# ZhangHH233/Retinal_OCT_Image_Segmentation_via_Deep_Learning

Measured on AMD Instinct MI355X. Metric: B-scans/sec (train fwd+bwd) at batch 32, 512x1024, higher is better.
Workload: dtype bf16; 1 GPU; SOTAS/Layers_Segment UNet(1,8,init_features=32) train step, 512x1024, batch 32/GPU (BASELINE configs[1]); global_batch=32, parallelism=dp1, hip_graph=False

## Files before the change

include/oct_hip.h:

```cpp
#ifndef OCT_HIP_H
#define OCT_HIP_H

#include <stddef.h>
#include <stdint.h>

#ifdef __cplusplus
extern "C" {
#endif

#define OCT_VERSION 220

#define OCT_DT_BF16 0
#define OCT_DT_F32 1

#define OCT_OK 0
#define OCT_IMG_SHIFT_ALL 2
#define OCT_E_INVALID (-22)
#define OCT_E_LAUNCH (-5)
#define OCT_E_NODEVICE (-19)

#define OCT_XF_NONE 0
#define OCT_XF_AFFINE_RELU 1
#define OCT_XF_AFFINE 2

// ... 69 lines not shown
  int kh, kw;
  int depth;
  int in_img_shift;
  int dy_img_mul, dy_img_add;
  int partials;
} OctWgradDesc;
typedef struct OctWgradArgs {
  const void* x0; const void* x1;
  const float* scale0; const float* shift0;
  const float* scale1; const float* shift1;
  const void* dy;
  float* dwp;
  float* dbias;
  const void* dy_y; const float* dy_coef; const float* dy_scale; const float* dy_shift;
  float* dbias_partials;
  void* dy_out;
} OctWgradArgs;
int oct_conv_wgrad(const OctWgradDesc* d, const OctWgradArgs* a, void* stream);
int oct_conv_wgrad_partials(const OctWgradDesc* d);
int oct_reduce_bias_partials(const float* part, int nparts, int rows, int channels, float* dbias, int accumulate,
                             void* stream);
int oct_conv_wgrad_fused_apply_ok(const OctWgradDesc* d);
int oct_conv_wgrad_apply_store_ok(const OctWgradDesc* d);
int oct_conv_wgrad_all_depth_taps_ok(const OctWgradDesc* d);
typedef struct OctConvBwdFusedArgs {
  const void* x;
  const float* scale; const float* shift;
  const float* mean; const float* invstd;
  const void* dy;
  const void* wpacked;
  void* dx;
  float* dwp;
  float* partials;
} OctConvBwdFusedArgs;
int oct_conv_backward_fused_ok(const OctWgradDesc* d);
int oct_conv_backward_fused_blocks(const OctWgradDesc* d);
int oct_conv_backward_fused(const OctWgradDesc* d, const OctConvBwdFusedArgs* a, void* stream);
int oct_unpack_wgrad(int mode, const float* dwp, float* grad, int cout, int cin, int accumulate, void* stream);
int oct_unpack_wgrad_kk(const float* dwp, float* grad, int cout, int cin, int kh, int kw, int accumulate, void* stream);
int oct_unpack_wgrad3d(int mode, const float* dwp, float* grad, int cout, int cin, int kdi, int accumulate, void* stream);
typedef struct OctUnpackJob {
  int mode, cout, cin, accumulate;
  int nparts, reserved;
  const float* dwp;
  float* grad;
} OctUnpackJob;
// ... 337 lines not shown
```

retinal_oct_image_segmentation_via_deep_learning_amd/_lib.py:

```python
from __future__ import annotations

import ctypes as C
import os
import subprocess
import threading

PKG_DIR = os.path.dirname(os.path.abspath(__file__))
LIB_PATH = os.environ.get("OCT_HIP_LIB") or os.path.join(PKG_DIR, "liboct_hip.so")
CSRC_DIR = os.path.join(PKG_DIR, "csrc")

DT_BF16, DT_F32 = 0, 1
XF_NONE, XF_AFFINE_RELU, XF_AFFINE = 0, 1, 2
IN_PLAIN, IN_S2D = 0, 1
IMG_SHIFT_ALL = 2
ACT_NONE, ACT_RELU, ACT_SIGMOID = 0, 1, 2
ACT_PRELU = 3
OUT_PLAIN, OUT_D2S = 0, 1
PACK_CONV_FPROP, PACK_CONV_DGRAD, PACK_DECONV_FPROP, PACK_DECONV_DGRAD, PACK_1X1_DGRAD, PACK_1X1_FPROP = range(6)
PACK_CONV3D_FPROP, PACK_CONV3D_DGRAD, PACK_DECONV3D_FPROP, PACK_DECONV3D_DGRAD = 6, 7, 8, 9
MAX_CLASSES = 16
HEAD_LOSS_SLOTS = 2 + 3 * MAX_CLASSES
SEG_NHWC, SEG_NCHW = 0, 1

c_void_p, c_int, c_size_t, c_float, c_double = C.c_void_p, C.c_int, C.c_size_t, C.c_float, C.c_double
# ... 120 lines not shown
    "oct_depth_pool_fwd": (c_int, [c_int, c_void_p, c_void_p, c_size_t, c_size_t, c_void_p]),
    "oct_depth_pool_bwd": (c_int, [c_int, c_void_p, c_void_p, c_void_p, c_size_t, c_size_t, c_void_p]),
    "oct_pack_weights_kk": (c_int, [c_int, c_int, c_void_p, c_void_p, c_int, c_int, c_int, c_int, c_void_p]),
    "oct_unpack_wgrad_kk": (c_int, [c_void_p, c_void_p, c_int, c_int, c_int, c_int, c_int, c_void_p]),
    "oct_affine_prelu_fwd": (c_int, [c_int, c_void_p, c_void_p, c_void_p, c_void_p, c_void_p, c_size_t, c_int, c_void_p]),
    "oct_affine_prelu_bwd": (c_int, [c_int, c_void_p, c_void_p, c_void_p, c_void_p, c_void_p, c_void_p, c_void_p, c_size_t,
                                     c_int, c_void_p]),
    "oct_maxpool_idx_fwd": (c_int, [c_int, c_void_p, c_void_p, c_void_p, c_int, c_int, c_int, c_int, c_int, c_void_p]),
    "oct_index_scatter": (c_int, [c_int, c_void_p, c_void_p, c_void_p, c_int, c_size_t, c_size_t, c_int, c_void_p]),
    "oct_index_gather": (c_int, [c_int, c_void_p, c_void_p, c_void_p, c_int, c_size_t, c_size_t, c_int, c_void_p]),
    "oct_prelu_bn_fused_ok": (c_int, [c_int, c_int]),
    "oct_dact_bn_reduce_prelu": (c_int, [c_int, c_void_p, c_void_p, c_void_p, c_void_p, c_void_p, c_void_p, c_void_p, c_void_p, c_void_p,
                                         c_int, c_int, c_int, c_int, c_void_p]),
    "oct_bn_bwd_apply_prelu_to": (c_int, [c_int, c_void_p, c_void_p, c_void_p, c_void_p, c_void_p, c_void_p, c_void_p, c_size_t, c_int,
                                          c_void_p]),
    "oct_maxpool_code_fwd": (c_int, [c_int, c_void_p, c_void_p, c_void_p, c_int, c_int, c_int, c_int, c_int, c_void_p]),
    "oct_window_scatter": (c_int, [c_int, c_void_p, c_void_p, c_void_p, c_int, c_int, c_int, c_int, c_int, c_void_p]),
    "oct_window_gather": (c_int, [c_int, c_void_p, c_void_p, c_void_p, c_int, c_int, c_int, c_int, c_int, c_void_p]),
    "oct_pack_weights_batch": (c_int, [c_int, c_int, C.POINTER(PackJob), c_void_p]),
    "oct_conv_forward": (c_int, [C.POINTER(ConvDesc), C.POINTER(ConvArgs), c_void_p]),
    "oct_conv_wgrad": (c_int, [C.POINTER(WgradDesc), C.POINTER(WgradArgs), c_void_p]),
    "oct_conv_wgrad_fused_apply_ok": (c_int, [C.POINTER(WgradDesc)]),
    "oct_conv_wgrad_apply_store_ok": (c_int, [C.POINTER(WgradDesc)]),
    "oct_conv_wgrad_all_depth_taps_ok": (c_int, [C.POINTER(WgradDesc)]),
    "oct_conv_backward_fused_ok": (c_int, [C.POINTER(WgradDesc)]),
    "oct_conv_backward_fused_blocks": (c_int, [C.POINTER(WgradDesc)]),
    "oct_conv_backward_fused": (c_int, [C.POINTER(WgradDesc), C.POINTER(ConvBwdFusedArgs), c_void_p]),
    "oct_conv_wgrad_partials": (c_int, [C.POINTER(WgradDesc)]),
    "oct_reduce_bias_partials": (c_int, [c_void_p, c_int, c_int, c_int, c_void_p, c_int, c_void_p]),
    "oct_unpack_wgrad": (c_int, [c_int, c_void_p, c_void_p, c_int, c_int, c_int, c_void_p]),
    "oct_unpack_wgrad_batch": (c_int, [c_int, C.POINTER(UnpackJob), c_void_p]),
    "oct_bn_finalize": (c_int, [c_void_p, c_int, c_int, c_double, c_void_p, c_void_p, c_float, c_float,
                                c_void_p, c_void_p, c_void_p, c_void_p, c_void_p, c_void_p, c_void_p, c_void_p]),
    "oct_bn_eval_coeffs": (c_int, [c_int, c_void_p, c_void_p, c_void_p, c_void_p, c_float, c_void_p, c_void_p,
                                   c_void_p, c_void_p]),
    "oct_bn_relu_pool_fwd": (c_int, [c_int, c_void_p, c_void_p, c_void_p, c_void_p, c_int, c_int, c_int, c_int,
                                     c_void_p]),
    "oct_bn_relu_fwd": (c_int, [c_int, c_void_p, c_void_p, c_void_p, c_void_p, c_size_t, c_int, c_void_p]),
    "oct_dact_bn_reduce": (c_int, [c_int, c_void_p, c_void_p, c_void_p, c_void_p, c_void_p, c_void_p, c_void_p,
                                   c_void_p, c_void_p, c_int, c_int, c_int, c_int, c_void_p]),
    "oct_dact_bn_reduce_blocks": (c_int, [c_int, c_int, c_int, c_int, c_int]),
    "oct_bn_bwd_apply_pool_ok": (c_int, [c_int, c_int, c_int, c_int, c_int]),
    "oct_bn_bwd_apply_pool": (c_int, [c_int, c_void_p, c_void_p, c_void_p, c_void_p, c_void_p, c_void_p, c_void_p,
                                      c_int, c_int, c_int, c_int, c_void_p]),
    "oct_bn_bwd_finalize": (c_int, [c_void_p, c_int, c_int, c_double, c_void_p, c_void_p, c_void_p, c_void_p,
                                    c_void_p, c_void_p, c_int, c_void_p]),
# ... 151 lines not shown
```

retinal_oct_image_segmentation_via_deep_learning_amd/csrc/common.h:

```cpp
#pragma once
#include <hip/hip_runtime.h>
#include <stdint.h>
#include <stddef.h>
#include "../../include/oct_hip.h"

typedef __bf16 bf16_t;
typedef float f32x16 __attribute__((ext_vector_type(16)));
typedef float f32x4 __attribute__((ext_vector_type(4)));
typedef __bf16 bf16x8 __attribute__((ext_vector_type(8)));
typedef __bf16 bf16x4 __attribute__((ext_vector_type(4)));
typedef unsigned int u32x4 __attribute__((ext_vector_type(4)));
typedef unsigned int u32x2 __attribute__((ext_vector_type(2)));

void oct_set_error(const char* fmt, ...);
#define OCT_CHECK(cond, ...)            \
  do {                                  \
    if (!(cond)) {                      \
      oct_set_error(__VA_ARGS__);       \
      return OCT_E_INVALID;             \
    }                                   \
  } while (0)
int oct_check_launch(const char* what);
int oct_lds_optin(const void* kernel, int bytes);
constexpr int OCT_LDS_CAP = 160 * 1024;
// ... 13 lines not shown
bool gemm1_plan(const OctConvDesc* d, ConvPlan* pl);
void igemm_plan(const OctConvDesc* d, ConvPlan* pl);
int launch_first(const ConvPlan& pl, const OctConvDesc* d, const OctConvArgs* a, hipStream_t s);
int launch_roll3d(const ConvPlan& pl, const OctConvDesc* d, const OctConvArgs* a, hipStream_t s);
int launch_igemm2(const ConvPlan& pl, const OctConvDesc* d, const OctConvArgs* a, hipStream_t s);
int launch_gemm1(const ConvPlan& pl, const OctConvDesc* d, const OctConvArgs* a, hipStream_t s);
int launch_igemm(const ConvPlan& pl, const OctConvDesc* d, const OctConvArgs* a, hipStream_t s);
bool igemm2_fused_plan(const OctWgradDesc* d, ConvPlan* pl);
int launch_igemm2_fused(const ConvPlan& pl, const OctWgradDesc* d, const OctConvBwdFusedArgs* a, hipStream_t s);

enum WgradPath { WGRAD_FIRST, WGRAD_W2, WGRAD_GENERIC };
struct WgradPlan {
  WgradPath path;
  int kernel;
  int cb, ib, th;
  int grid;
  int slabs;
  bool all_depth_taps;
};
bool first_wgrad_plan(const OctWgradDesc* d, bool dbias, bool dy_coef, WgradPlan* pl);
bool wgrad2_plan(const OctWgradDesc* d, WgradPlan* pl);
void wgrad_plan(const OctWgradDesc* d, WgradPlan* pl);
bool wgrad2_apply_store_ok(const OctWgradDesc* d, const WgradPlan& pl);
int launch_first_wgrad(const WgradPlan& pl, const OctWgradDesc* d, const OctWgradArgs* a, hipStream_t s);
int launch_wgrad2(const WgradPlan& pl, const OctWgradDesc* d, const OctWgradArgs* a, hipStream_t s);
int launch_wgrad(const WgradPlan& pl, const OctWgradDesc* d, const OctWgradArgs* a, hipStream_t s);

__device__ __forceinline__ float xf_floor(int xf) { return xf == 2 ? -__builtin_inff() : 0.f; }
__device__ __forceinline__ float to_f32(float v) { return v; }
__device__ __forceinline__ float to_f32(bf16_t v) { return (float)v; }
template <typename T> __device__ __forceinline__ T from_f32(float v);
template <> __device__ __forceinline__ float from_f32<float>(float v) { return v; }
template <> __device__ __forceinline__ bf16_t from_f32<bf16_t>(float v) { return (bf16_t)v; }
__device__ __forceinline__ unsigned pack_bf16x2(float a, float b) {
  typedef __bf16 bf16x2 __attribute__((ext_vector_type(2)));
  bf16x2 v;
  v[0] = (bf16_t)a;
  v[1] = (bf16_t)b;
  return __builtin_bit_cast(unsigned, v);
}
__device__ __forceinline__ float bf16lo(unsigned u) { return __uint_as_float(u << 16); }
__device__ __forceinline__ float bf16hi(unsigned u) { return __uint_as_float(u & 0xffff0000u); }

template <typename T, int V> struct alignas((sizeof(T) * V) > 16 ? 16 : (sizeof(T) * V)) VecT { T v[V]; };

template <typename T, int V>
// ... 179 lines not shown
```

retinal_oct_image_segmentation_via_deep_learning_amd/csrc/conv_dispatch.hip:

```cpp
#include "common.h"
#include <stdlib.h>

static bool v2_enabled() {
  static const bool on = [] { const char* e = getenv("OCT_DISABLE_V2"); return !(e && e[0] == '1'); }();
  return on;
}

static ConvPlan plan_conv_forward(const OctConvDesc* d) {
  ConvPlan pl = {};
  if (v2_enabled()) {
    if (first_plan(d, &pl) || roll3d_plan(d, &pl)) return pl;
    if (igemm2_plan(d, &pl)) {
      gemm1_plan(d, &pl);
      return pl;
    }
  }
  igemm_plan(d, &pl);
  return pl;
}

static WgradPlan plan_conv_wgrad(const OctWgradDesc* d, bool dbias, bool dy_coef) {
  WgradPlan pl = {};
  if (v2_enabled() && (first_wgrad_plan(d, dbias, dy_coef, &pl) || wgrad2_plan(d, &pl))) return pl;
  wgrad_plan(d, &pl);
// ... 93 lines not shown
  OCT_CHECK(!(d->xform1 && (!a->scale1 || !a->shift1)), "oct_conv_wgrad: xform1 without scale/shift");
  OCT_CHECK(!d->partials || !a->dbias || a->dbias_partials, "oct_conv_wgrad: partials mode with a bias gradient needs dbias_partials");
  const bool apply_store = a->dy_coef && a->dy_out;
  OCT_CHECK(!a->dy_out || a->dy_coef, "oct_conv_wgrad: dy_out goes with dy_coef");
  OCT_CHECK(!apply_store || oct_conv_wgrad_apply_store_ok(d),
            "oct_conv_wgrad: dy_coef + dy_out is not available for this descriptor (oct_conv_wgrad_apply_store_ok)");
  OCT_CHECK(!apply_store || !a->dbias, "oct_conv_wgrad: dy_coef + dy_out takes no bias gradient");
  const WgradPlan pl = plan_conv_wgrad(d, a->dbias != nullptr, a->dy_coef != nullptr && !apply_store);
  OCT_CHECK(!a->dy_coef || apply_store || pl.path == WGRAD_FIRST, "oct_conv_wgrad: the fused BN-backward apply is only implemented for the 1->F first layer in bf16");
  OCT_CHECK(!a->dy_coef || (a->dy_y && a->dy_scale && a->dy_shift), "oct_conv_wgrad: fused apply needs y, scale, shift");
  if (d->partials) {
    const int slabs = plan_conv_wgrad(d, false, false).slabs;
    OCT_CHECK(pl.slabs == slabs, "oct_conv_wgrad: with these arguments the launch writes %d partial slabs, oct_conv_wgrad_partials "
              "answered %d (first layer with a bias gradient?)", pl.slabs, slabs);
  }
  hipStream_t s = as_stream(stream);
  switch (pl.path) {
    case WGRAD_FIRST: return launch_first_wgrad(pl, d, a, s);
    case WGRAD_W2: return launch_wgrad2(pl, d, a, s);
    default: return launch_wgrad(pl, d, a, s);
  }
}

static bool plan_conv_backward_fused(const OctWgradDesc* d, ConvPlan* pl) {
  return d && v2_enabled() && igemm2_fused_plan(d, pl);
}

extern "C" int oct_conv_backward_fused_ok(const OctWgradDesc* d) {
  ConvPlan pl;
  return plan_conv_backward_fused(d, &pl) ? 1 : 0;
}

extern "C" int oct_conv_backward_fused_blocks(const OctWgradDesc* d) {
  ConvPlan pl;
  return plan_conv_backward_fused(d, &pl) ? pl.stat_rows : 0;
}

extern "C" int oct_conv_backward_fused(const OctWgradDesc* d, const OctConvBwdFusedArgs* a, void* stream) {
  OCT_CHECK(d && a, "oct_conv_backward_fused: null descriptor");
  ConvPlan pl;
  OCT_CHECK(plan_conv_backward_fused(d, &pl),
            "oct_conv_backward_fused: not available for this descriptor (oct_conv_backward_fused_ok): bf16, 2-D, 3x3, c0 = cout = 32, "
            "c1 = 0, BN + ReLU on load, w %% 32 == 0, h %% 8 == 0, atomics mode");
  OCT_CHECK(a->x && a->scale && a->shift && a->mean && a->invstd && a->dy && a->wpacked && a->dx && a->dwp && a->partials,
            "oct_conv_backward_fused: null tensor");
  return launch_igemm2_fused(pl, d, a, as_stream(stream));
// ... 2 lines not shown
```

retinal_oct_image_segmentation_via_deep_learning_amd/csrc/wgrad2.hip:

```cpp
#include "common.h"

#include <type_traits>

struct Wgrad2Params {
  const bf16_t* x0; const bf16_t* x1;
  const float* sc0; const float* sh0; const float* sc1; const float* sh1;
  const bf16_t* dy; float* dwp; float* dbias;
  int n, h, w, c0, c1, ktot, cout, xf0, xf1, dy_mode;
  int tiles_x, tiles_y, ntiles, per_wg;
  int interleave;
  int depth, img_shift;
  int dy_mul, dy_add;
  int part_mode; size_t slab_elems; float* dbias_part;
  int ty0, pad_y, nstore;
  unsigned long long* trace;
  const bf16_t* dy_y; const float* dy_coef; const float* dy_sc; const float* dy_sh; bf16_t* dy_out;
};

#ifdef OCT_TRACE
#define W2TRACE(slot, idx)                                                                                     \
  do {                                                                                                         \
    if (p.trace && blockIdx.x == 0 && blockIdx.y == 0 && blockIdx.z == 0 && (threadIdx.x & 63) == 0 && (idx) < 256) \
      p.trace[(slot) * 256 + (idx)] = __builtin_amdgcn_s_memtime();                                            \
  } while (0)
// ... 64 lines not shown
    const bool second = cg >= p.c0;
    const bool xf = second ? (p.xf1 != 0) : (p.xf0 != 0);
    sxf[i] = xf ? (second ? p.sc1[cg - p.c0] : p.sc0[cg]) : 1.f;
    sxf[32 * IB + i] = xf ? (second ? p.sh1[cg - p.c0] : p.sh0[cg]) : 0.f;
  }
  float* const sdy = reinterpret_cast<float*>(smem + w2_sdy(TAPS, CB, IB, TH));
  if constexpr (DYAPPLY) {
    for (int i = tid; i < 32 * CB; i += 512) {
      const int ch = co_sb + i;
      sdy[i] = p.dy_coef[ch]; sdy[32 * CB + i] = p.dy_coef[p.cout + ch]; sdy[2 * 32 * CB + i] = p.dy_coef[2 * p.cout + ch];
      sdy[3 * 32 * CB + i] = p.dy_sc[ch]; sdy[4 * 32 * CB + i] = p.dy_sh[ch];
    }
  }
  __syncthreads();

  if (wave >= 4) {
    const int ptid = tid - 256, g = ptid & 3, pb = ptid >> 2;
    constexpr int SIB = (NPI * 4 + 255) / 256;
    constexpr int SDB = (NPD * 4 + 255) / 256;
    constexpr int D = DRING;
    typedef typename std::conditional<DYAPPLY, W2StageY<CB, SDB>, W2NoY>::type StageY;
    struct Stage { u32x4 ri[IB][SIB]; u32x4 rd[CB][SDB]; unsigned vm[IB]; unsigned vd; int img, tyi, txi; StageY yy; };
    Stage R[D];
    int reli[SIB], reld[SDB];
    int lyv[RSH ? SIB : 1];
    unsigned code[SIB], dcode[SDB];
#pragma unroll
    for (int j = 0; j < SIB; ++j) {
      const int pix = pb + 64 * j;
      const int ly = pix / LW, lx = pix - ly * LW;
      reli[j] = (RSH ? ly + p.ty0 : ly) * p.w + lx;
      if constexpr (RSH) lyv[j] = ly;
      const int ylast = p.h - (p.tiles_y - 1) * TH + HALO_Y, xlast = p.w - (p.tiles_x - 1) * TW + HALO;
      unsigned c = pix >= NPI ? 16u : 0u;
      if (HALO) c |= ((!RSH && HALO_Y && ly == 0) ? 1u : 0u) | (lx == 0 ? 4u : 0u);
      c |= ((!RSH && ly >= ylast) ? 2u : 0u) | (lx >= xlast ? 8u : 0u);
      code[j] = c | (SWZ ? (unsigned)(((lx >> 3) & 1) << 1) << 8 : 0u);
    }
    unsigned dswz[SDB];
#pragma unroll
    for (int j = 0; j < SDB; ++j) {
      const int pix = pb + 64 * j;
      const int ly = pix / TW, lx = pix - ly * TW;
      dswz[j] = SWZ ? (unsigned)(((lx >> 3) & 1) << 1) : 0u;
      reld[j] = (p.dy_mode == OCT_IN_S2D) ? (2 * ly) * (2 * p.w) + 2 * lx : ly * p.w + lx;
      dcode[j] = RAGGED ? ((ly >= p.h - (p.tiles_y - 1) * TH ? 2u : 0u) | (lx >= p.w - (p.tiles_x - 1) * TW ? 8u : 0u)) : 0u;
    }
    auto issue = [&](int s, Stage& S) {
      int t = t0 + s * tstep;
      const int txi = t % p.tiles_x; t /= p.tiles_x;
      const int tyi = t % p.tiles_y; const int img = t / p.tiles_y;
      const unsigned edge = 16u | (tyi == 0 ? 1u : 0u) | (tyi == p.tiles_y - 1 ? 2u : 0u) | (txi == 0 ? 4u : 0u) |
                            (txi == p.tiles_x - 1 ? 8u : 0u);
      const size_t origin = ((size_t)img * p.h + tyi * TH) * p.w + txi * TW;
      S.img = img; S.tyi = tyi; S.txi = txi;
      int ylo = 0; unsigned ynum = 0;
      if constexpr (RSH) {
        const int ytop = tyi * TH - p.pad_y + p.ty0;
        ylo = max(0, -ytop);
        ynum = (unsigned)max(0, min(LH, p.h - ytop) - ylo);
      }
      bool zok = true;
      size_t in_origin = origin;
      if (D3 && p.depth > 0) {
        const int dz = img % p.depth + p.img_shift;
        zok = dz >= 0 && dz < p.depth;
        if (zok) in_origin = ((size_t)(img + p.img_shift) * p.h + tyi * TH) * p.w + txi * TW;
      }
#pragma unroll
      for (int blk = 0; blk < IB; ++blk) {
        const int cg = ci_sb + blk * 32;
        const bool second = cg >= p.c0;
        const int cs = second ? p.c1 : p.c0;
        const bf16_t* base = second ? p.x1 + in_origin * p.c1 + (cg - p.c0) : p.x0 + in_origin * p.c0 + cg;
        const unsigned corner = RSH ? (unsigned)(p.pad_y * p.w + HALO) : (unsigned)(HALO * (p.w + 1));
        const unsigned cs2 = 2u * (unsigned)cs, safe = corner * cs2 + (unsigned)g * 16u;
        const unsigned char* const hb = reinterpret_cast<const unsigned char*>(base) - (size_t)corner * cs2;
        unsigned vm = 0;
#pragma unroll
        for (int j = 0; j < SIB; ++j) {
          bool ok = (!D3 || zok) && (code[j] & edge) == 0;
          if constexpr (RSH) ok = ok && (unsigned)(lyv[j] - ylo) < ynum;
          S.ri[blk][j] = *reinterpret_cast<const u32x4*>(hb + (ok ? __umul24((unsigned)reli[j], cs2) + (unsigned)g * 16u : safe));
          vm |= ok ? (1u << j) : 0u;
        }
        S.vm[blk] = vm;
      }
#pragma unroll
      for (int blk = 0; blk < CB; ++blk) {
        const int row = co_sb + blk * 32;
        const bf16_t* base;
        int cs;
        if (p.dy_mode == OCT_IN_S2D) {
          cs = p.cout >> 2;
          const int dydx = row / cs, co = row - dydx * cs;
          const int img2 = (D3 && p.dy_mul) ? img * p.dy_mul + p.dy_add : img;
          const size_t o2 = ((size_t)img2 * (2 * p.h) + 2 * tyi * TH + (dydx >> 1)) * (size_t)(2 * p.w) + 2 * txi * TW + (dydx & 1);
          base = p.dy + o2 * cs + co;
        } else {
          cs = p.cout;
          base = p.dy + origin * cs + row;
        }
        const unsigned cs2 = 2u * (unsigned)cs;
        const unsigned char* const db = reinterpret_cast<const unsigned char*>(base);
        unsigned vd = 0;
#pragma unroll
        for (int j = 0; j < SDB; ++j) {
          const bool ok = !RAGGED || (dcode[j] & edge) == 0;
          S.rd[blk][j] = *reinterpret_cast<const u32x4*>(db + ((ok ? __umul24((unsigned)reld[j], cs2) : 0u) + (unsigned)g * 16u));
          vd |= ok ? (1u << j) : 0u;
        }
        if (RAGGED) S.vd = vd;
        if constexpr (DYAPPLY) {
          const unsigned char* const yb = reinterpret_cast<const unsigned char*>(p.dy_y + origin * cs + row);
#pragma unroll
          for (int j = 0; j < SDB; ++j)
            S.yy.ry[blk][j] = *reinterpret_cast<const u32x4*>(yb + (__umul24((unsigned)reld[j], cs2) + (unsigned)g * 16u));
          if (blk == 0) S.yy.ob = reinterpret_cast<const unsigned char*>(p.dy_out + origin * cs + co_sb);
        }
      }
    };
    auto commit = [&](unsigned char* buf, const Stage& S, const bool st) {
#pragma unroll
      for (int blk = 0; blk < IB; ++blk) {
        const int cg = ci_sb + blk * 32;
        const bool second = cg >= p.c0;
        const bool xf = second ? (p.xf1 != 0) : (p.xf0 != 0);
        const float flo = xf_floor(second ? p.xf1 : p.xf0);
        float s[8], b[8];
        if (xf) {
          const float* sc = sxf + blk * 32 + g * 8;
          const float* sh = sxf + 32 * IB + blk * 32 + g * 8;
          const f32x4 s0 = *reinterpret_cast<const f32x4*>(sc), s1 = *reinterpret_cast<const f32x4*>(sc + 4);
          const f32x4 b0 = *reinterpret_cast<const f32x4*>(sh), b1 = *reinterpret_cast<const f32x4*>(sh + 4);
#pragma unroll
          for (int j = 0; j < 4; ++j) { s[j] = s0[j]; s[4 + j] = s1[j]; b[j] = b0[j]; b[4 + j] = b1[j]; }
        }
#pragma unroll
        for (int j = 0; j < SIB; ++j) {
          if ((code[j] & 16u) == 0) {
            u32x4 v = S.ri[blk][j];
            if (xf) {
#pragma unroll
              for (int e = 0; e < 4; ++e) {
                const float lo = fmaxf(fmaf(__uint_as_float(v[e] << 16), s[2 * e], b[2 * e]), flo);
// ... 4 lines not shown
            const bool live = ((S.vm[blk] >> j) & 1u) != 0;
#pragma unroll
            for (int e = 0; e < 4; ++e) v[e] = live ? v[e] : 0u;
            *reinterpret_cast<u32x4*>(buf + blk * INB + (pb + 64 * j) * 64 + ((unsigned)g ^ ((code[j] >> 8) & 3u)) * 16) = v;
          }
        }
      }
#pragma unroll
      for (int blk = 0; blk < CB; ++blk) {
        float k0[8], k1[8], k2[8], ysc[8], ysh[8];
        if constexpr (DYAPPLY) {
          const float* const t = sdy + blk * 32 + g * 8;
#pragma unroll
          for (int q = 0; q < 2; ++q) {
            const f32x4 a0 = *reinterpret_cast<const f32x4*>(t + 4 * q), a1 = *reinterpret_cast<const f32x4*>(t + 32 * CB + 4 * q);
            const f32x4 a2 = *reinterpret_cast<const f32x4*>(t + 2 * 32 * CB + 4 * q), a3 = *reinterpret_cast<const f32x4*>(t + 3 * 32 * CB + 4 * q);
            const f32x4 a4 = *reinterpret_cast<const f32x4*>(t + 4 * 32 * CB + 4 * q);
#pragma unroll
            for (int e = 0; e < 4; ++e) { k0[4 * q + e] = a0[e]; k1[4 * q + e] = a1[e]; k2[4 * q + e] = a2[e]; ysc[4 * q + e] = a3[e]; ysh[4 * q + e] = a4[e]; }
          }
        }
#pragma unroll
        for (int j = 0; j < SDB; ++j) {
          u32x4 v = S.rd[blk][j];
          if constexpr (DYAPPLY) {
            const u32x4 yv = S.yy.ry[blk][j];
#pragma unroll
            for (int e = 0; e < 4; ++e) {
              const float ya = bf16lo(yv[e]), yb = bf16hi(yv[e]);
              const float ga = fmaf(ya, ysc[2 * e], ysh[2 * e]) > 0.f ? bf16lo(v[e]) : 0.f;
              const float gb = fmaf(yb, ysc[2 * e + 1], ysh[2 * e + 1]) > 0.f ? bf16hi(v[e]) : 0.f;
              v[e] = pack_bf16x2(fmaf(k0[2 * e], ga, fmaf(k1[2 * e], ya, k2[2 * e])),
                                 fmaf(k0[2 * e + 1], gb, fmaf(k1[2 * e + 1], yb, k2[2 * e + 1])));
            }
            if (st) *reinterpret_cast<u32x4*>(const_cast<unsigned char*>(S.yy.ob) + (size_t)blk * 64 +
                                              (__umul24((unsigned)reld[j], 2u * (unsigned)p.cout) + (unsigned)g * 16u)) = v;
          }
          if (RAGGED) {
            const bool live = ((S.vd >> j) & 1u) != 0;
#pragma unroll
            for (int e = 0; e < 4; ++e) v[e] = live ? v[e] : 0u;
          }
          *reinterpret_cast<u32x4*>(buf + IB * INB + blk * DYB + (pb + 64 * j) * 64 + ((unsigned)g ^ dswz[j]) * 16) = v;
        }
      }
    };
    const int last = nstage - 1;
#pragma unroll
    for (int j = 0; j < D; ++j) issue(min(j, last), R[j]);
    commit(stage0, R[0], true);
    issue(min(D, last), R[0]);
    __syncthreads();
    for (int s0 = 0; s0 < nstage_pad; s0 += D) {
#pragma unroll
      for (int j = 0; j < D; ++j) {
        const int nx = s0 + j + 1;
        if (wave == 4) W2TRACE(4, nx - 1);
        commit(stage0 + (nx & 1) * STAGEB, R[(j + 1) % D], nx <= last);
        if (wave == 4) W2TRACE(5, nx - 1);
        issue(min(nx + D, last), R[(j + 1) % D]);
        if (wave == 4) W2TRACE(6, nx - 1);
        __syncthreads();
        if (wave == 4) W2TRACE(7, nx - 1);
      }
    }
    return;
  }

  __builtin_amdgcn_s_setprio(3);
  const int pair = MULTI ? 0 : wave % PAIRS, psx = MULTI ? 0 : wave / PAIRS;
  const int cb = MULTI ? (wave >> 1) * WCB : pair / IB, ib = MULTI ? (wave & 1) * WIB : pair % IB;
  const int g4 = lane >> 4, li = lane & 15;
  const int lane_off = W16 ? (8 * g4 + (li >> 2)) * 64 + (4 * (li & 3)) * 2
                           : (8 * (g4 >> 1) + (li >> 2)) * 64 + (16 * (g4 & 1) + 4 * (li & 3)) * 2;
  int lo1[2], lo2[2][2];
#pragma unroll
  for (int h = 0; h < 2; ++h) {
    lo1[h] = lane_off + ((h ^ (g4 & 1)) * 32);
#pragma unroll
    for (int tx = 1; tx <= 2; ++tx) {
      const int carry = ((tx + (li >> 2) + 4) >> 3) & 1;
      lo2[tx - 1][h] = lane_off + 4 * 64 + ((h ^ (g4 & 1) ^ carry) * 32);
    }
// ... 239 lines not shown
    else if (pairs && nco % 2 == 0) cb = 2;
    else th = 16;
  } else {
    const bool m_ok = nco % 4 == 0 && (d->h % 4) == 0 && d->depth == 0 && d->dy_img_mul == 0;
    if (m_ok && nci % 4 == 0) { cb = ib = 4; th = 4; }
    else if (m_ok && nci % 2 == 0) { cb = 4; ib = 2; th = 4; }
    else if (big) cb = ib = 2;
  }
  pl->path = WGRAD_W2;
  pl->cb = cb; pl->ib = ib; pl->th = th;
  pl->slabs = w2_grid(d->taps == 1 ? 1 : 9, cb, ib, th, nco, nci, d->n, d->h, d->w).gx * (cb * ib > 4 ? 1 : 4 / (cb * ib));
  return true;
}

bool wgrad2_apply_store_ok(const OctWgradDesc* d, const WgradPlan& pl) {
  if (pl.path != WGRAD_W2 || d->taps != 9 || d->kh == 7 || d->depth > 0 || d->dy_img_mul != 0 || d->dy_mode != OCT_IN_PLAIN || d->partials)
    return false;
  if ((d->w % 32) != 0 || (d->h % pl.th) != 0) return false;
  const int nco = d->cout / 32, nci = (d->c0 + d->c1) / 32;
  if (nco / pl.cb != 1 || nci / pl.ib != 1) return false;
  return pl.cb == 1 && pl.ib == 2 && pl.th == 8;
}

int launch_wgrad2(const WgradPlan& pl, const OctWgradDesc* d, const OctWgradArgs* a, hipStream_t s) {
  const int ktot = d->c0 + d->c1;
  Wgrad2Params p;
  p.dy_y = (const bf16_t*)a->dy_y; p.dy_coef = a->dy_coef; p.dy_sc = a->dy_scale; p.dy_sh = a->dy_shift; p.dy_out = (bf16_t*)a->dy_out;
  p.x0 = (const bf16_t*)a->x0; p.x1 = (const bf16_t*)a->x1;
  p.sc0 = a->scale0; p.sh0 = a->shift0; p.sc1 = a->scale1; p.sh1 = a->shift1;
  p.dy = (const bf16_t*)a->dy; p.dwp = a->dwp; p.dbias = a->dbias;
#ifdef OCT_TRACE
  p.trace = g_trace_w2;
#else
  p.trace = nullptr;
#endif
  p.part_mode = d->partials ? 1 : 0;
  p.slab_elems = (size_t)d->taps * d->cout * ktot; p.dbias_part = a->dbias_partials;
  p.n = d->n; p.h = d->h; p.w = d->w; p.c0 = d->c0; p.c1 = d->c1; p.ktot = ktot; p.cout = d->cout;
  p.xf0 = d->xform0; p.xf1 = d->xform1; p.dy_mode = d->dy_mode;
  p.depth = d->depth; p.img_shift = d->in_img_shift; p.dy_mul = d->dy_img_mul; p.dy_add = d->dy_img_add;
  const int nco = d->cout / 32, nci = ktot / 32;
  p.ty0 = 0; p.pad_y = 1; p.nstore = 9;
  int rc = OCT_OK;
  if (d->kh == 7) {
    const bool whole = (p.w % 32) == 0 && (p.h % 8) == 0;
    float* const dwp0 = p.dwp;
    for (int ty0 = 0; ty0 < 7 && rc == OCT_OK; ty0 += 3) {
      p.ty0 = ty0; p.pad_y = 3; p.nstore = ty0 == 6 ? 3 : 9;
      p.dwp = dwp0 + (size_t)ty0 * 3 * d->cout * ktot;
      if (ty0 > 0) p.dbias = nullptr;
      if (ty0 == 6) rc = whole ? launch_w2r<3, 2, 2, 8, false, false, true>(p, nco, nci, s) : launch_w2r<3, 2, 2, 8, true, false, true>(p, nco, nci, s);
      else rc = whole ? launch_w2r<9, 2, 2, 8, false, false, true>(p, nco, nci, s) : launch_w2r<9, 2, 2, 8, true, false, true>(p, nco, nci, s);
    }
  } else if (a->dy_coef) {
    rc = launch_w2r<9, 1, 2, 8, false, false, false, true>(p, nco, nci, s);
  } else if (d->taps == 9) {
    if (pl.cb == 2 && pl.ib == 2) rc = launch_w2<9, 2, 2, 8>(p, nco, nci, s);
    else if (pl.ib == 2) rc = launch_w2<9, 1, 2, 8>(p, nco, nci, s);
    else if (pl.cb == 2) rc = launch_w2<9, 2, 1, 8>(p, nco, nci, s);
    else rc = launch_w2<9, 1, 1, 16>(p, nco, nci, s);
  } else {
    if (pl.cb == 4 && pl.ib == 4) rc = launch_w2<1, 4, 4, 4>(p, nco, nci, s);
    else if (pl.cb == 4) rc = launch_w2<1, 4, 2, 4>(p, nco, nci, s);
    else if (pl.cb == 2) rc = launch_w2<1, 2, 2, 8>(p, nco, nci, s);
    else rc = launch_w2<1, 1, 1, 8>(p, nco, nci, s);
  }
  return rc ? rc : oct_check_launch("wgrad2");
}
```

retinal_oct_image_segmentation_via_deep_learning_amd/engine.py:

```python
from __future__ import annotations

import ctypes as C
import os
from dataclasses import dataclass, field

import torch

from . import _lib as L

BN_EPS = 1e-5
BN_MOMENTUM = 0.1

@dataclass
class ConvKeys:
    w: str
    bn: str
    b: str | None = None


@dataclass
class BlockSpec:
    name: str
    c1: ConvKeys
    c2: ConvKeys
# ... 227 lines not shown
                        _xf(src.bn0), _xf(src.bn1), dy_mode, kh, kw, depth, in_shift,
                        dy_img[0], dy_img[1], parts)
        bias_parts = None
        if parts:
            nparts = L.lib().oct_conv_wgrad_partials(C.byref(d))
            dwp = torch.empty((nparts, taps, cout, ktot), dtype=torch.float32, device=dy.device)
            dwp._oct_nparts = nparts
            if dbias is not None:
                bias_parts = torch.empty((nparts, cout), dtype=torch.float32, device=dy.device)
        elif dwp is None:
            dwp = self._dwp_take(taps * cout * ktot, dy.device).view(taps, cout, ktot)
        a = L.WgradArgs(L.ptr(src.x0), L.ptr(src.x1),
                        L.ptr(src.bn0.scale) if src.bn0 else None, L.ptr(src.bn0.shift) if src.bn0 else None,
                        L.ptr(src.bn1.scale) if src.bn1 else None, L.ptr(src.bn1.shift) if src.bn1 else None,
                        L.ptr(dy), L.ptr(dwp), L.ptr(dbias), *([L.ptr(t) for t in fused_apply] if fused_apply
                                                                 else [None, None, None, None]), L.ptr(bias_parts), L.ptr(dy_out))
        ev = self._prof_begin()
        L.check(L.lib().oct_conv_wgrad(C.byref(d), C.byref(a), _stream()), "oct_conv_wgrad")
        self._prof_end(ev, "wgrad", (taps, ktot, cout, n, h, w, dy_mode, 0))
        if bias_parts is not None:
            L.check(L.lib().oct_reduce_bias_partials(bias_parts.data_ptr(), nparts, cout,
                                                     cout // 4 if dy_mode == L.IN_S2D else cout, dbias.data_ptr(), 1,
                                                     _stream()), "oct_reduce_bias_partials")
        return dwp

    def _dwp_take(self, numel: int, dev) -> torch.Tensor:
        if self._arena_on:
            lo = self._arena_off
            self._arena_off = lo + (numel + 63) // 64 * 64
            if self._arena is not None and self._arena_off <= self._arena.numel() and self._arena.device == dev:
                return self._arena[lo:lo + numel]
            self._arena_short = True
        return torch.zeros(numel, dtype=torch.float32, device=dev)

    def _arena_begin(self, dev):
        self._arena_on, self._arena_off, self._arena_short = True, 0, False
        self._unpack_jobs = []
        if self._arena is not None and self._arena.device == dev:
            self._arena.zero_()

    def _flush_unpack(self):
        if self._unpack_jobs:
            arr = (L.UnpackJob * len(self._unpack_jobs))(*[j[0] for j in self._unpack_jobs])
            L.check(L.lib().oct_unpack_wgrad_batch(len(self._unpack_jobs), arr, _stream()), "oct_unpack_wgrad_batch")
            self._unpack_jobs = []

# ... 174 lines not shown
        if defer_apply and not pooled:
            return g, coef
        if pool_fused:
            L.check(lib.oct_bn_bwd_apply_pool(self.dt, L.ptr(da), dpool.data_ptr(), rec.y.data_ptr(), rec.bn.scale.data_ptr(),
                                              rec.bn.shift.data_ptr(), coef.data_ptr(), g.data_ptr(), n, h, w, c, _stream()),
                    "oct_bn_bwd_apply_pool")
            return g
        if head_dl is not None:
            hd, dl8, hw = head_dl
            L.check(lib.oct_head_bwd_apply(C.byref(hd), dl8.data_ptr(), rec.y.data_ptr(), rec.bn.scale.data_ptr(),
                                           rec.bn.shift.data_ptr(), hw.data_ptr(), coef.data_ptr(), g.data_ptr(), _stream()),
                    "oct_head_bwd_apply")
            return g
        L.check(lib.oct_bn_bwd_apply(self.dt, g.data_ptr(), rec.y.data_ptr(), coef.data_ptr(),
                                     None if pooled else rec.bn.scale.data_ptr(),
                                     None if pooled else rec.bn.shift.data_ptr(), n * h * w, c, _stream()),
                "oct_bn_bwd_apply")
        if self.debug is not None:
            self.debug["dy:" + rec.wkey] = g.float().clone()
            self.debug["y:" + rec.wkey] = rec.y.float().clone()
            self.debug["coef:" + rec.wkey] = coef.clone()
        return g

    def _wgrad_applies(self, rec: ConvRec) -> bool:
        if self.wgrad_apply_off or self.debug is not None or self.deterministic:
            return False
        src = rec.src
        d = L.WgradDesc(self.dt, rec.n, rec.h, rec.w, src.c0, src.c1, rec.cout, 9, _xf(src.bn0), _xf(src.bn1), L.IN_PLAIN)
        return bool(L.lib().oct_conv_wgrad_apply_store_ok(C.byref(d)))

    def _conv_backward(self, rec: ConvRec, dy, G, accumulate, need_dx=True, apply_coef=None):
        n, h, w = rec.n, rec.h, rec.w
        src = rec.src
        cin = src.channels
        if apply_coef is not None:
            dwp = self._wgrad(src, dy, rec.cout, 9, n, h, w, fused_apply=(rec.y, apply_coef, rec.bn.scale, rec.bn.shift), dy_out=dy)
        else:
            dwp = self._wgrad(src, dy, rec.cout, 9, n, h, w)
        self._unpack(L.PACK_CONV_FPROP, dwp, G[rec.wkey], rec.cout, cin, accumulate)
        if not need_dx:
            return None, None
        wp = self._pack(rec.wkey, self._P[rec.wkey], L.PACK_CONV_DGRAD, rec.cout, cin)
        d0 = self._act(n, h, w, src.c0, dy.device)
        d1 = self._act(n, h, w, src.c1, dy.device) if src.c1 else None
        self._conv(Src(dy, rec.cout), wp, cin, 9, n, h, w, d0, y1=d1, split=src.c0 if src.c1 else 0)
        if self.debug is not None:
            def bnc(b):
                return None if b is None else (b.scale.clone(), b.shift.clone())
            self.debug["layer:" + rec.wkey] = dict(
                x0=src.x0.float().clone(), bn0=bnc(src.bn0), x1=None if src.x1 is None else src.x1.float().clone(),
                bn1=bnc(src.bn1), dy=dy.float().clone(), d0=d0.float().clone(), d1=None if d1 is None else d1.float().clone(),
                y=rec.y.float().clone())
        return d0, d1

    def _conv_backward_fused(self, r1: ConvRec, r2: ConvRec, dy2, G, accumulate):
        src = r2.src
        if self.fused_bwd_off or self.debug is not None or self.deterministic or src.c1 or src.bn0 is None or src.bn0 is not r1.bn or src.x0 is not r1.y:
            return None
        lib = L.lib()
        n, h, w, cin, cout = r2.n, r2.h, r2.w, src.c0, r2.cout
        d = L.WgradDesc(self.dt, n, h, w, cin, 0, cout, 9, _xf(src.bn0), L.XF_NONE, L.IN_PLAIN, 0, 0, 0, 0, 0, 0, 0)
        if not lib.oct_conv_backward_fused_ok(C.byref(d)):
            return None
        dev = dy2.device
        wp = self._pack(r2.wkey, self._P[r2.wkey], L.PACK_CONV_DGRAD, cout, cin)
        da1 = self._act(n, h, w, cin, dev)
        dwp = self._dwp_take(9 * cout * cin, dev).view(9, cout, cin)
        parts = torch.empty((lib.oct_conv_backward_fused_blocks(C.byref(d)), 2, cin), dtype=torch.float32, device=dev)
        a = L.ConvBwdFusedArgs(L.ptr(r1.y), L.ptr(r1.bn.scale), L.ptr(r1.bn.shift), L.ptr(r1.bn.mean), L.ptr(r1.bn.invstd),
                               L.ptr(dy2), L.ptr(wp), L.ptr(da1), L.ptr(dwp), L.ptr(parts))
        ev = self._prof_begin()
        L.check(lib.oct_conv_backward_fused(C.byref(d), C.byref(a), _stream()), "oct_conv_backward_fused")
        self._prof_end(ev, "igemm", (9, cout, cin, n, h, w, L.IN_PLAIN, L.OUT_PLAIN))
        self._unpack(L.PACK_CONV_FPROP, dwp, G[r2.wkey], cout, cin, accumulate)
        return da1, parts

    def _block_backward(self, name, da, dpool, G, accumulate, need_dx=True, partials=None, head_dl=None):
        r1, r2 = self._ctx.convs[name]
        for r in (r1, r2):
            if r.cbkey and not accumulate and not r.bn.frozen:
                G[r.cbkey].zero_()
        dy2 = self._bn_backward(r2, da, dpool, G, accumulate, partials=partials, head_dl=head_dl)
        fused = self._conv_backward_fused(r1, r2, dy2, G, accumulate)
        if fused is not None:
            da1, parts1 = fused
        else:
            (da1, _), parts1 = self._conv_backward(r2, dy2, G, accumulate), None
        first_fused = False
        if not need_dx and r1.src.c1 == 0 and r1.src.bn0 is None:
            qd = L.WgradDesc(self.dt, r1.n, r1.h, r1.w, r1.src.c0, 0, r1.cout, 9, L.XF_NONE, L.XF_NONE, L.IN_PLAIN)
            first_fused = bool(L.lib().oct_conv_wgrad_fused_apply_ok(C.byref(qd)))
        if first_fused:
            da1, coef = self._bn_backward(r1, da1, None, G, accumulate, partials=parts1, defer_apply=True)
            dwp = self._wgrad(r1.src, da1, r1.cout, 9, r1.n, r1.h, r1.w,
                              fused_apply=(r1.y, coef, r1.bn.scale, r1.bn.shift))
            self._unpack(L.PACK_CONV_FPROP, dwp, G[r1.wkey], r1.cout, 1, accumulate)
            return None, None
        if self._wgrad_applies(r1):
            da1, coef = self._bn_backward(r1, da1, None, G, accumulate, partials=parts1, defer_apply=True)
            return self._conv_backward(r1, da1, G, accumulate, need_dx=need_dx, apply_coef=coef)
        dy1 = self._bn_backward(r1, da1, None, G, accumulate, partials=parts1)
        return self._conv_backward(r1, dy1, G, accumulate, need_dx=need_dx)

    def backward_stages(self):
        sp = self.spec

        def blk_keys(b: BlockSpec):
            ks = []
            for c in (b.c1, b.c2):
                ks += [c.w, c.bn + ".weight", c.bn + ".bias"] + ([c.b] if c.b else [])
            return ks
        nd = len(sp.dec)
        stages = []
        for di in range(nd - 1, -1, -1):
            ks = ([sp.head_w, sp.head_b] if di == nd - 1 else []) + blk_keys(sp.dec[di]) + list(sp.ups[di][:2])
            stages.append((f"dec{di}", ks))
        for li in range(len(sp.enc) - 1, -1, -1):
            stages.append((f"enc{li}", blk_keys(sp.enc[li])))
        return stages

    def _stage_done(self, hook, idx):
        if hook is not None and idx in hook.flush_stages:
            self._flush_unpack()
# ... 115 lines not shown
```

Before: 1257 B-scans/s.

## Fuse BN-backward apply into wgrad for wider cout tiles (apply_to path)

Adds an 'apply_to' variant of the wgrad2 kernel that applies the deferred BN-backward coefficients to dY inside the weight-gradient kernel for cb=2 tilings, writing the applied dY to a separate or in-place buffer. It splits dY staging from input staging so the applied dY is stored only by the z==0 column of blocks, and it uses a shallower dY pipeline depth when CB==2. The engine routes the second conv of blocks, and first convs that qualify, through this path, which avoids a separate BN-apply pass over the activation gradient. The cost is extra register pressure and possibly an extra buffer allocation when cin>64.

```diff
diff --git a/include/oct_hip.h b/include/oct_hip.h
--- a/include/oct_hip.h
+++ b/include/oct_hip.h
@@ -115,6 +115,8 @@
                              void* stream);
 int oct_conv_wgrad_fused_apply_ok(const OctWgradDesc* d);
 int oct_conv_wgrad_apply_store_ok(const OctWgradDesc* d);
+int oct_conv_wgrad_apply_to_ok(const OctWgradDesc* d);
+int oct_conv_wgrad_apply_to(const OctWgradDesc* d, const OctWgradArgs* a, void* stream);
 int oct_conv_wgrad_all_depth_taps_ok(const OctWgradDesc* d);
 typedef struct OctConvBwdFusedArgs {
   const void* x;
diff --git a/retinal_oct_image_segmentation_via_deep_learning_amd/_lib.py b/retinal_oct_image_segmentation_via_deep_learning_amd/_lib.py
--- a/retinal_oct_image_segmentation_via_deep_learning_amd/_lib.py
+++ b/retinal_oct_image_segmentation_via_deep_learning_amd/_lib.py
@@ -166,6 +166,8 @@
     "oct_conv_wgrad": (c_int, [C.POINTER(WgradDesc), C.POINTER(WgradArgs), c_void_p]),
     "oct_conv_wgrad_fused_apply_ok": (c_int, [C.POINTER(WgradDesc)]),
     "oct_conv_wgrad_apply_store_ok": (c_int, [C.POINTER(WgradDesc)]),
+    "oct_conv_wgrad_apply_to_ok": (c_int, [C.POINTER(WgradDesc)]),
+    "oct_conv_wgrad_apply_to": (c_int, [C.POINTER(WgradDesc), C.POINTER(WgradArgs), c_void_p]),
     "oct_conv_wgrad_all_depth_taps_ok": (c_int, [C.POINTER(WgradDesc)]),
     "oct_conv_backward_fused_ok": (c_int, [C.POINTER(WgradDesc)]),
     "oct_conv_backward_fused_blocks": (c_int, [C.POINTER(WgradDesc)]),
diff --git a/retinal_oct_image_segmentation_via_deep_learning_amd/csrc/common.h b/retinal_oct_image_segmentation_via_deep_learning_amd/csrc/common.h
--- a/retinal_oct_image_segmentation_via_deep_learning_amd/csrc/common.h
+++ b/retinal_oct_image_segmentation_via_deep_learning_amd/csrc/common.h
@@ -59,6 +59,8 @@
 bool wgrad2_plan(const OctWgradDesc* d, WgradPlan* pl);
 void wgrad_plan(const OctWgradDesc* d, WgradPlan* pl);
 bool wgrad2_apply_store_ok(const OctWgradDesc* d, const WgradPlan& pl);
+bool wgrad2_apply_to_ok(const OctWgradDesc* d, const WgradPlan& pl);
+int wgrad2_apply_to_zcols(const OctWgradDesc* d, const WgradPlan& pl);
 int launch_first_wgrad(const WgradPlan& pl, const OctWgradDesc* d, const OctWgradArgs* a, hipStream_t s);
 int launch_wgrad2(const WgradPlan& pl, const OctWgradDesc* d, const OctWgradArgs* a, hipStream_t s);
 int launch_wgrad(const WgradPlan& pl, const OctWgradDesc* d, const OctWgradArgs* a, hipStream_t s);
diff --git a/retinal_oct_image_segmentation_via_deep_learning_amd/csrc/conv_dispatch.hip b/retinal_oct_image_segmentation_via_deep_learning_amd/csrc/conv_dispatch.hip
--- a/retinal_oct_image_segmentation_via_deep_learning_amd/csrc/conv_dispatch.hip
+++ b/retinal_oct_image_segmentation_via_deep_learning_amd/csrc/conv_dispatch.hip
@@ -139,6 +139,36 @@
   }
 }
 
+extern "C" int oct_conv_wgrad_apply_to_ok(const OctWgradDesc* d) {
+  int kh, kw;
+  if (!d || d->dtype != OCT_DT_BF16 || !kernel_size(d->taps, d->kh, d->kw, &kh, &kw)) return 0;
+  if (d->n <= 0 || d->h <= 0 || d->w <= 0 || d->c0 <= 0 || d->c1 < 0 || d->cout <= 0) return 0;
+  return wgrad2_apply_to_ok(d, plan_conv_wgrad(d, false, false)) ? 1 : 0;
+}
+
+extern "C" int oct_conv_wgrad_apply_to(const OctWgradDesc* d, const OctWgradArgs* a, void* stream) {
+  OCT_CHECK(d && a, "oct_conv_wgrad_apply_to: null descriptor");
+  OCT_CHECK(oct_conv_wgrad_apply_to_ok(d),
+            "oct_conv_wgrad_apply_to: not available for this descriptor (oct_conv_wgrad_apply_to_ok): bf16, 2-D, 3x3, plain dY, "
+            "w %% 32 == 0, h %% 8 == 0, atomics mode, cout %% 64 == 0");
+  OCT_CHECK(a->x0 && a->dy && a->dwp, "oct_conv_wgrad_apply_to: null tensor");
+  OCT_CHECK(d->c1 == 0 || a->x1, "oct_conv_wgrad_apply_to: c1 > 0 but x1 is null");
+  OCT_CHECK(d->xform0 >= 0 && d->xform0 <= OCT_XF_AFFINE && d->xform1 >= 0 && d->xform1 <= OCT_XF_AFFINE, "oct_conv_wgrad_apply_to: bad xform");
+  OCT_CHECK(!(d->xform0 && (!a->scale0 || !a->shift0)), "oct_conv_wgrad_apply_to: xform0 without scale/shift");
+  OCT_CHECK(!(d->xform1 && (!a->scale1 || !a->shift1)), "oct_conv_wgrad_apply_to: xform1 without scale/shift");
+  OCT_CHECK(a->dy_coef && a->dy_y && a->dy_scale && a->dy_shift && a->dy_out, "oct_conv_wgrad_apply_to: needs dy_y, dy_coef, dy_scale, dy_shift and dy_out");
+  OCT_CHECK(!a->dbias && !a->dbias_partials, "oct_conv_wgrad_apply_to: takes no bias gradient");
+  OCT_CHECK((size_t)d->n * d->h * d->w < (1u << 31), "oct_conv_wgrad_apply_to: too many pixels");
+  const WgradPlan pl = plan_conv_wgrad(d, false, false);
+  const size_t bytes = (size_t)d->n * d->h * d->w * d->cout * 2;
+  const char* const in = (const char*)a->dy; const char* const out = (const char*)a->dy_out;
+  const bool apart = out + bytes <= in || in + bytes <= out;
+  OCT_CHECK(apart || (out == in && wgrad2_apply_to_zcols(d, pl) == 1),
+            "oct_conv_wgrad_apply_to: dy_out overlaps dy; in place (dy_out == dy) is only for a single input-channel column, "
+            "this launch has %d", wgrad2_apply_to_zcols(d, pl));
+  return launch_wgrad2(pl, d, a, as_stream(stream));
+}
+
 static bool plan_conv_backward_fused(const OctWgradDesc* d, ConvPlan* pl) {
   return d && v2_enabled() && igemm2_fused_plan(d, pl);
 }
diff --git a/retinal_oct_image_segmentation_via_deep_learning_amd/csrc/wgrad2.hip b/retinal_oct_image_segmentation_via_deep_learning_amd/csrc/wgrad2.hip
--- a/retinal_oct_image_segmentation_via_deep_learning_amd/csrc/wgrad2.hip
+++ b/retinal_oct_image_segmentation_via_deep_learning_amd/csrc/wgrad2.hip
@@ -110,6 +110,7 @@
     typedef typename std::conditional<DYAPPLY, W2StageY<CB, SDB>, W2NoY>::type StageY;
     struct Stage { u32x4 ri[IB][SIB]; u32x4 rd[CB][SDB]; unsigned vm[IB]; unsigned vd; int img, tyi, txi; StageY yy; };
     Stage R[D];
+    constexpr int DD = (DYAPPLY && CB == 2) ? 1 : D;
     int reli[SIB], reld[SDB];
     int lyv[RSH ? SIB : 1];
     unsigned code[SIB], dcode[SDB];
@@ -134,7 +135,7 @@
       reld[j] = (p.dy_mode == OCT_IN_S2D) ? (2 * ly) * (2 * p.w) + 2 * lx : ly * p.w + lx;
       dcode[j] = RAGGED ? ((ly >= p.h - (p.tiles_y - 1) * TH ? 2u : 0u) | (lx >= p.w - (p.tiles_x - 1) * TW ? 8u : 0u)) : 0u;
     }
-    auto issue = [&](int s, Stage& S) {
+    auto issue_in = [&](int s, Stage& S) {
       int t = t0 + s * tstep;
       const int txi = t % p.tiles_x; t /= p.tiles_x;
       const int tyi = t % p.tiles_y; const int img = t / p.tiles_y;
@@ -174,6 +175,14 @@
         }
         S.vm[blk] = vm;
       }
+    };
+    auto issue_d = [&](int s, Stage& S) {
+      int t = t0 + s * tstep;
+      const int txi = t % p.tiles_x; t /= p.tiles_x;
+      const int tyi = t % p.tiles_y; const int img = t / p.tiles_y;
+      const unsigned edge = 16u | (tyi == 0 ? 1u : 0u) | (tyi == p.tiles_y - 1 ? 2u : 0u) | (txi == 0 ? 4u : 0u) |
+                            (txi == p.tiles_x - 1 ? 8u : 0u);
+      const size_t origin = ((size_t)img * p.h + tyi * TH) * p.w + txi * TW;
 #pragma unroll
       for (int blk = 0; blk < CB; ++blk) {
         const int row = co_sb + blk * 32;
@@ -208,7 +217,8 @@
         }
       }
     };
-    auto commit = [&](unsigned char* buf, const Stage& S, const bool st) {
+    auto issue = [&](int s, Stage& S, int sd, Stage& SD) { issue_in(s, S); issue_d(sd, SD); };
+    auto commit = [&](unsigned char* buf, const Stage& S, const Stage& SD, const bool st) {
 #pragma unroll
       for (int blk = 0; blk < IB; ++blk) {
         const int cg = ci_sb + blk * 32;
@@ -259,9 +269,9 @@
         }
 #pragma unroll
         for (int j = 0; j < SDB; ++j) {
-          u32x4 v = S.rd[blk][j];
+          u32x4 v = SD.rd[blk][j];
           if constexpr (DYAPPLY) {
-            const u32x4 yv = S.yy.ry[blk][j];
+            const u32x4 yv = SD.yy.ry[blk][j];
 #pragma unroll
             for (int e = 0; e < 4; ++e) {
               const float ya = bf16lo(yv[e]), yb = bf16hi(yv[e]);
@@ -270,11 +280,11 @@
               v[e] = pack_bf16x2(fmaf(k0[2 * e], ga, fmaf(k1[2 * e], ya, k2[2 * e])),
                                  fmaf(k0[2 * e + 1], gb, fmaf(k1[2 * e + 1], yb, k2[2 * e + 1])));
             }
-            if (st) *reinterpret_cast<u32x4*>(const_cast<unsigned char*>(S.yy.ob) + (size_t)blk * 64 +
+            if (st) *reinterpret_cast<u32x4*>(const_cast<unsigned char*>(SD.yy.ob) + (size_t)blk * 64 +
                                               (__umul24((unsigned)reld[j], 2u * (unsigned)p.cout) + (unsigned)g * 16u)) = v;
           }
           if (RAGGED) {
-            const bool live = ((S.vd >> j) & 1u) != 0;
+            const bool live = ((SD.vd >> j) & 1u) != 0;
 #pragma unroll
             for (int e = 0; e < 4; ++e) v[e] = live ? v[e] : 0u;
           }
@@ -283,19 +293,23 @@
       }
     };
     const int last = nstage - 1;
-#pragma unroll
-    for (int j = 0; j < D; ++j) issue(min(j, last), R[j]);
-    commit(stage0, R[0], true);
-    issue(min(D, last), R[0]);
+    const bool stcol = blockIdx.z == 0;
+#pragma unroll
+    for (int j = 0; j < D; ++j) {
+      issue_in(min(j, last), R[j]);
+      if (j < DD) issue_d(min(j, last), R[j]);
+    }
+    commit(stage0, R[0], R[0], stcol);
+    issue(min(D, last), R[0], min(DD, last), R[0]);
     __syncthreads();
     for (int s0 = 0; s0 < nstage_pad; s0 += D) {
 #pragma unroll
       for (int j = 0; j < D; ++j) {
         const int nx = s0 + j + 1;
         if (wave == 4) W2TRACE(4, nx - 1);
-        commit(stage0 + (nx & 1) * STAGEB, R[(j + 1) % D], nx <= last);
+        commit(stage0 + (nx & 1) * STAGEB, R[(j + 1) % D], R[(j + 1) % DD], nx <= last && stcol);
         if (wave == 4) W2TRACE(5, nx - 1);
-        issue(min(nx + D, last), R[(j + 1) % D]);
+        issue(min(nx + D, last), R[(j + 1) % D], min(nx + DD, last), R[(j + 1) % DD]);
         if (wave == 4) W2TRACE(6, nx - 1);
         __syncthreads();
         if (wave == 4) W2TRACE(7, nx - 1);
@@ -581,6 +595,16 @@
   return pl.cb == 1 && pl.ib == 2 && pl.th == 8;
 }
 
+static constexpr int W2_APPLY_TO_MAX_ZCOLS = 1, W2_APPLY_TO_MAX_YCOLS = 2;
+int wgrad2_apply_to_zcols(const OctWgradDesc* d, const WgradPlan& pl) { return (d->c0 + d->c1) / 32 / pl.ib; }
+bool wgrad2_apply_to_ok(const OctWgradDesc* d, const WgradPlan& pl) {
+  if (pl.path != WGRAD_W2 || d->taps != 9 || d->kh == 7 || d->depth > 0 || d->dy_img_mul != 0 || d->dy_mode != OCT_IN_PLAIN || d->partials)
+    return false;
+  if (d->dtype != OCT_DT_BF16 || (d->w % 32) != 0 || (d->h % pl.th) != 0) return false;
+  if (pl.cb != 2 || pl.th != 8 || (pl.ib != 1 && pl.ib != 2)) return false;
+  return wgrad2_apply_to_zcols(d, pl) <= W2_APPLY_TO_MAX_ZCOLS && d->cout / 32 / pl.cb <= W2_APPLY_TO_MAX_YCOLS;
+}
+
 int launch_wgrad2(const WgradPlan& pl, const OctWgradDesc* d, const OctWgradArgs* a, hipStream_t s) {
   const int ktot = d->c0 + d->c1;
   Wgrad2Params p;
@@ -612,7 +636,9 @@
       else rc = whole ? launch_w2r<9, 2, 2, 8, false, false, true>(p, nco, nci, s) : launch_w2r<9, 2, 2, 8, true, false, true>(p, nco, nci, s);
     }
   } else if (a->dy_coef) {
-    rc = launch_w2r<9, 1, 2, 8, false, false, false, true>(p, nco, nci, s);
+    if (pl.cb == 2 && pl.ib == 2) rc = launch_w2r<9, 2, 2, 8, false, false, false, true>(p, nco, nci, s);
+    else if (pl.cb == 2) rc = launch_w2r<9, 2, 1, 8, false, false, false, true>(p, nco, nci, s);
+    else rc = launch_w2r<9, 1, 2, 8, false, false, false, true>(p, nco, nci, s);
   } else if (d->taps == 9) {
     if (pl.cb == 2 && pl.ib == 2) rc = launch_w2<9, 2, 2, 8>(p, nco, nci, s);
     else if (pl.ib == 2) rc = launch_w2<9, 1, 2, 8>(p, nco, nci, s);
diff --git a/retinal_oct_image_segmentation_via_deep_learning_amd/engine.py b/retinal_oct_image_segmentation_via_deep_learning_amd/engine.py
--- a/retinal_oct_image_segmentation_via_deep_learning_amd/engine.py
+++ b/retinal_oct_image_segmentation_via_deep_learning_amd/engine.py
@@ -273,6 +273,20 @@
             L.check(L.lib().oct_reduce_bias_partials(bias_parts.data_ptr(), nparts, cout,
                                                      cout // 4 if dy_mode == L.IN_S2D else cout, dbias.data_ptr(), 1,
                                                      _stream()), "oct_reduce_bias_partials")
+        return dwp
+
+    def _wgrad_apply_to(self, rec: ConvRec, da, coef, dy_out):
+        src, n, h, w, cout = rec.src, rec.n, rec.h, rec.w, rec.cout
+        d = L.WgradDesc(self.dt, n, h, w, src.c0, src.c1, cout, 9, _xf(src.bn0), _xf(src.bn1), L.IN_PLAIN)
+        dwp = self._dwp_take(9 * cout * src.channels, da.device).view(9, cout, src.channels)
+        a = L.WgradArgs(L.ptr(src.x0), L.ptr(src.x1),
+                        L.ptr(src.bn0.scale) if src.bn0 else None, L.ptr(src.bn0.shift) if src.bn0 else None,
+                        L.ptr(src.bn1.scale) if src.bn1 else None, L.ptr(src.bn1.shift) if src.bn1 else None,
+                        L.ptr(da), L.ptr(dwp), None, L.ptr(rec.y), L.ptr(coef), L.ptr(rec.bn.scale), L.ptr(rec.bn.shift), None,
+                        L.ptr(dy_out))
+        ev = self._prof_begin()
+        L.check(L.lib().oct_conv_wgrad_apply_to(C.byref(d), C.byref(a), _stream()), "oct_conv_wgrad_apply_to")
+        self._prof_end(ev, "wgrad", (9, src.channels, cout, n, h, w, L.IN_PLAIN, 0))
         return dwp
 
     def _dwp_take(self, numel: int, dev) -> torch.Tensor:
@@ -493,18 +507,25 @@
             self.debug["coef:" + rec.wkey] = coef.clone()
         return g
 
-    def _wgrad_applies(self, rec: ConvRec) -> bool:
+    def _wgrad_applies(self, rec: ConvRec):
         if self.wgrad_apply_off or self.debug is not None or self.deterministic:
-            return False
+            return None
         src = rec.src
         d = L.WgradDesc(self.dt, rec.n, rec.h, rec.w, src.c0, src.c1, rec.cout, 9, _xf(src.bn0), _xf(src.bn1), L.IN_PLAIN)
-        return bool(L.lib().oct_conv_wgrad_apply_store_ok(C.byref(d)))
-
-    def _conv_backward(self, rec: ConvRec, dy, G, accumulate, need_dx=True, apply_coef=None):
+        if L.lib().oct_conv_wgrad_apply_store_ok(C.byref(d)):
+            return "store"
+        return "to" if L.lib().oct_conv_wgrad_apply_to_ok(C.byref(d)) else None
+
+    def _conv_backward(self, rec: ConvRec, dy, G, accumulate, need_dx=True, apply_coef=None, apply_form="store"):
         n, h, w = rec.n, rec.h, rec.w
         src = rec.src
         cin = src.channels
-        if apply_coef is not None:
+        if apply_coef is not None and apply_form == "to":
+            da = dy
+            if cin > 64:
+                dy = self._act(n, h, w, rec.cout, da.device)
+            dwp = self._wgrad_apply_to(rec, da, apply_coef, dy)
+        elif apply_coef is not None:
             dwp = self._wgrad(src, dy, rec.cout, 9, n, h, w, fused_apply=(rec.y, apply_coef, rec.bn.scale, rec.bn.shift), dy_out=dy)
         else:
             dwp = self._wgrad(src, dy, rec.cout, 9, n, h, w)
@@ -551,12 +572,17 @@
         for r in (r1, r2):
             if r.cbkey and not accumulate and not r.bn.frozen:
                 G[r.cbkey].zero_()
-        dy2 = self._bn_backward(r2, da, dpool, G, accumulate, partials=partials, head_dl=head_dl)
-        fused = self._conv_backward_fused(r1, r2, dy2, G, accumulate)
-        if fused is not None:
-            da1, parts1 = fused
+        form2 = self._wgrad_applies(r2) if (dpool is None and head_dl is None and da is not None) else None
+        if form2 == "to":
+            da2, coef2 = self._bn_backward(r2, da, None, G, accumulate, partials=partials, defer_apply=True)
+            (da1, _), parts1 = self._conv_backward(r2, da2, G, accumulate, apply_coef=coef2, apply_form="to"), None
         else:
-            (da1, _), parts1 = self._conv_backward(r2, dy2, G, accumulate), None
+            dy2 = self._bn_backward(r2, da, dpool, G, accumulate, partials=partials, head_dl=head_dl)
+            fused = self._conv_backward_fused(r1, r2, dy2, G, accumulate)
+            if fused is not None:
+                da1, parts1 = fused
+            else:
+                (da1, _), parts1 = self._conv_backward(r2, dy2, G, accumulate), None
         first_fused = False
         if not need_dx and r1.src.c1 == 0 and r1.src.bn0 is None:
             qd = L.WgradDesc(self.dt, r1.n, r1.h, r1.w, r1.src.c0, 0, r1.cout, 9, L.XF_NONE, L.XF_NONE, L.IN_PLAIN)
@@ -567,9 +593,10 @@
                               fused_apply=(r1.y, coef, r1.bn.scale, r1.bn.shift))
             self._unpack(L.PACK_CONV_FPROP, dwp, G[r1.wkey], r1.cout, 1, accumulate)
             return None, None
-        if self._wgrad_applies(r1):
+        form1 = self._wgrad_applies(r1)
+        if form1 is not None:
             da1, coef = self._bn_backward(r1, da1, None, G, accumulate, partials=parts1, defer_apply=True)
-            return self._conv_backward(r1, da1, G, accumulate, need_dx=need_dx, apply_coef=coef)
+            return self._conv_backward(r1, da1, G, accumulate, need_dx=need_dx, apply_coef=coef, apply_form=form1)
         dy1 = self._bn_backward(r1, da1, None, G, accumulate, partials=parts1)
         return self._conv_backward(r1, dy1, G, accumulate, need_dx=need_dx)
 
```

Result: no change. 1261 B-scans/s, median of 6 (+0.3%).
